# rainerzufalldererste/simd_dct

Hardware: AMD Instinct MI355X
Metric: Mpixels/s 8x8 fwd+inv int16 DCT, 8192x8192 plane (higher is better)
Workload: dtype f32

## Files before the change

simd_dct_amd/csrc/batch_plan.h:

```cpp
#ifndef MDCT_BATCH_PLAN_H
#define MDCT_BATCH_PLAN_H

#include <stddef.h>
#include <stdint.h>

#include <vector>

#include "mdct.h"

#if defined(__HIPCC__)
#define MDCT_HD __host__ __device__ __forceinline__
#else
#define MDCT_HD inline
#endif

namespace mdct
{

struct BatchDesc
{
  const void *from;
  void *to;
  uint64_t pitch_in, pitch_out;
  uint32_t bpr;
  uint32_t tiles;
  uint32_t tiles_m, tiles_s;
  uint32_t first;
  uint32_t table;
  uint32_t has_lut;
  uint32_t rows;
};
static_assert(sizeof(BatchDesc) == 64, "one s_load_dwordx16");
constexpr uint32_t kDescLut = 1, kDescPaired = 2;

struct MagicDiv
{
  uint32_t m, s;
};
inline MagicDiv magic_div(uint32_t d)
{
  if (d <= 1)
    return MagicDiv{0, 0};
  uint32_t l = 0;
  while ((1ull << l) < d)
    l++;
  const uint64_t m = ((1ull << 32) * ((1ull << l) - d)) / d + 1;
  return MagicDiv{(uint32_t)m, 1u | ((l - 1) << 8)};
}
MDCT_HD uint32_t magic_apply(uint32_t n, uint32_t m, uint32_t s)
{
  const uint32_t t = (uint32_t)(((uint64_t)n * m) >> 32);
  return (t + ((n - t) >> (s & 0xFF))) >> (s >> 8);
}

constexpr int kBatchChain = 8;
constexpr uint32_t kBatchMaxTiles = 0xFFFFFFFFu / 64;

template <class FirstOf>
MDCT_HD uint32_t batch_plane_of(uint32_t w, uint32_t n, uint32_t uniform, uint32_t pp_m, uint32_t pp_s, const uint32_t (&first8)[kBatchChain], FirstOf first_of)
{
  if (uniform)
    return magic_apply(w, pp_m, pp_s);
  uint32_t p = 0;
  for (int i = 1; i < kBatchChain; i++)
    p += w >= first8[i] ? 1u : 0u;
  if (n > (uint32_t)kBatchChain)
  {
    uint32_t lo = 0, hi = n;
    while (hi - lo > 1)
    {
      const uint32_t mid = (lo + hi) >> 1;
      if (first_of(mid) <= w)
        lo = mid;
      else
        hi = mid;
    }
    p = lo;
  }
  return p;
}

struct BatchLayout
{
  std::vector<BatchDesc> descs;
  std::vector<int> plane;
  std::vector<int> tables;
  uint32_t total = 0;
  uint32_t uniform = 0;
  uint32_t per_plane = 0;
  MagicDiv pp{0, 0};
  uint32_t first8[kBatchChain];
  int with_lut = 0;
  int consumed = 0;
};

inline uint64_t batch_tiles_of(uint64_t bpr, uint64_t rows, bool paired)
{
  return paired ? (rows / 2) * (bpr / 32) + (rows & 1) * ((bpr + 63) / 64) : ((bpr + 63) / 64) * rows;
}

struct BatchPos
{
  uint32_t row, b0, s, straddle;
};
MDCT_HD BatchPos batch_pos(uint32_t lt, uint32_t bpr, uint32_t tiles, uint32_t tiles_m, uint32_t tiles_s, uint32_t flags, uint32_t rows)
{
  const uint32_t u = magic_apply(lt, tiles_m, tiles_s), blk0 = (lt - u * tiles) * 64;
  BatchPos p;
  if (!(flags & kDescPaired))
  {
    p.row = u;
    p.b0 = blk0;
    p.s = bpr - blk0 < 64u ? bpr - blk0 : 64u;
    p.straddle = 0;
    return p;
  }
  const uint32_t second = blk0 >= bpr ? 1u : 0u;
  p.row = 2 * u + second;
  p.b0 = second ? blk0 - bpr : blk0;
  p.s = bpr - p.b0 < 64u ? bpr - p.b0 : 64u;
  p.straddle = (!second && p.s < 64u && p.row + 1 < rows) ? 1u : 0u;
  return p;
}

template <class Plane>
inline void batch_layout(const Plane *planes, const int *table_id, const unsigned char *has_lut, int i0, int n, size_t blob_bytes, size_t table_size, BatchLayout &out,
                         bool pair_rows = false)
{
  out = BatchLayout();
  uint64_t run = 0;
  for (int i = i0; i < n; i++)
  {
    const Plane &p = planes[i];
    const uint64_t bpr = p.sizeX / 8, rows = p.sizeY / 8;
    if (bpr == 0 || rows == 0)
    {
      out.consumed++;
      continue;
    }
    const bool paired = pair_rows && bpr % 64 == 32 && rows >= 2 && (uint64_t)p.pitch_in < (1ull << 26) && (uint64_t)p.pitch_out < (1ull << 26);
    const uint64_t tiles = paired ? bpr / 32 : (bpr + 63) / 64;
    if (bpr > 0xFFFFFFFFull || rows > 0xFFFFFFFFull || ((bpr + 63) / 64) * rows / rows != (bpr + 63) / 64)
      break;
    const uint64_t mine = batch_tiles_of(bpr, rows, paired);
    if (run + mine > kBatchMaxTiles)
      break;
    int slot = -1;
    bool new_table = false;
    if (table_id[i] >= 0)
    {
      for (size_t k = 0; k < out.tables.size() && slot < 0; k++)
        if (out.tables[k] == table_id[i])
          slot = (int)k;
      new_table = slot < 0;
      if (new_table)
        slot = (int)out.tables.size();
    }
    if (blob_bytes && (out.tables.size() + (new_table ? 1 : 0)) * table_size + (out.descs.size() + 1) * sizeof(BatchDesc) > blob_bytes)
      break;
    if (new_table)
      out.tables.push_back(table_id[i]);
    BatchDesc d;
    d.from = p.from;
    d.to = p.to;
    d.pitch_in = p.pitch_in;
    d.pitch_out = p.pitch_out;
    d.bpr = (uint32_t)bpr;
    d.tiles = (uint32_t)tiles;
    const MagicDiv md = magic_div(d.tiles);
    d.tiles_m = md.m;
    d.tiles_s = md.s;
    d.first = (uint32_t)run;
    d.table = slot < 0 ? 0u : (uint32_t)(slot * table_size);
    d.has_lut = (has_lut[i] ? kDescLut : 0u) | (paired ? kDescPaired : 0u);
    d.rows = (uint32_t)rows;
    out.with_lut += has_lut[i] ? 1 : 0;
    out.descs.push_back(d);
    out.plane.push_back(i);
    out.consumed++;
    run += mine;
  }
  out.total = (uint32_t)run;
  const size_t nd = out.descs.size();
  out.uniform = nd > 0;
  auto tiles_of = [&](size_t k) { return batch_tiles_of(out.descs[k].bpr, out.descs[k].rows, (out.descs[k].has_lut & kDescPaired) != 0); };
  for (size_t k = 1; k < nd; k++)
    if (tiles_of(k) != tiles_of(0))
      out.uniform = 0;
  out.per_plane = out.uniform ? (uint32_t)tiles_of(0) : 0;
  out.pp = magic_div(out.per_plane);
  for (int k = 0; k < kBatchChain; k++)
    out.first8[k] = (size_t)k < nd ? out.descs[k].first : 0xFFFFFFFFu;
}

struct BatchWhere
{
  uint32_t p, row, tile;
  BatchPos pos;
};
inline BatchWhere batch_locate(const BatchDesc *descs, uint32_t n, uint32_t uniform, MagicDiv pp, const uint32_t (&first8)[kBatchChain], uint32_t w)
{
  const uint32_t p = batch_plane_of(w, n, uniform, pp.m, pp.s, first8, [descs](uint32_t k) { return descs[k].first; });
  const BatchDesc &d = descs[p];
  const BatchPos pos = batch_pos(w - d.first, d.bpr, d.tiles, d.tiles_m, d.tiles_s, d.has_lut, d.rows);
  return BatchWhere{p, pos.row, pos.b0 / 64, pos};
}

}
#endif
```

simd_dct_amd/csrc/mdct_api.hip:

```cpp
#include <hip/hip_runtime.h>

#include <cmath>
#include <cstdarg>
#include <cstdio>
#include <cstring>
#include <cxxabi.h>
#include <dlfcn.h>
#include <cstdlib>
#include <string>
#include <mutex>
#include <type_traits>
#include <unordered_map>
#include <vector>

#include "mdct.h"
#include "mdct_kernels.h"
#include "own_tables.h"

namespace
{

thread_local char g_err[512] = "";

int fail(int code, const char *fmt, ...)
// ... 607 lines not shown
        return fail(MDCT_INVALID_PARAMETER, "output strip pitch %zu must be >= 8*sizeX = %zu and a multiple of 16", p.pitch_out, 8 * p.sizeX);
      const uintptr_t in0 = (uintptr_t)p.from, in1 = in0 + (p.sizeY ? (p.sizeY - 1) * p.pitch_in + p.sizeX : 0);
      const uintptr_t out0 = (uintptr_t)p.to, out1 = out0 + (p.sizeY >= 8 ? (p.sizeY / 8 - 1) * p.pitch_out + 8 * p.sizeX : 0);
      if (in0 < out1 && out0 < in1)
        return fail(MDCT_INVALID_PARAMETER, "plane %d: the q32 product cannot be written over its own input (to overlaps from)", i);
      float q[64];
      q32_pair_table(p.lut, false, q);
      q32_safe = q32_safe || table_needs_safe(q);
    }
  for (int i = 0; i < n; i++)
  {
    const Plane &p = planes[i];
    int r;
    if constexpr (U8 || GEN)
      r = u8_plane_args(p.from, p.to, p.pitch_in, p.pitch_out, p.sizeX, p.sizeY, 0, p.sizeY / 8);
    else
      r = own_plane_args(p.from, p.to, sizeof(int16_t), p.pitch_in, p.pitch_out, p.sizeX, p.sizeY, 0, p.sizeY / 8);
    if (r)
      return r;
    if constexpr (GEN)
    {
      const bool fwd = mode == kModeFwdU8;
      if ((((uintptr_t)(fwd ? p.to : p.from)) | ((fwd ? p.pitch_out : p.pitch_in) * sizeof(int16_t))) & 15)
        return fail(MDCT_INVALID_PARAMETER, "coefficient rows must be 16-byte aligned");
    }
    in.has_lut[i] = p.lut != nullptr;
    in.bounded[i] = q32 ? !q32_safe : (U8 ? u8_table_is_tame(p.lut) : (GEN ? (mode == kModeFwdU8 && u8_table_is_bounded(p.lut)) : lut_bounded(p.lut)));
    if (rt && !p.lut)
      continue;
    int id = -1;
    for (size_t k = 0; k < src.size() && id < 0; k++)
      if (src[k] == p.lut || (src[k] && p.lut && memcmp(src[k], p.lut, 64 * sizeof(float)) == 0))
        id = (int)k;
    if (id < 0)
    {
      mdct::OwnTables tb;
      if (q32)
      {
        memset(&tb, 0, sizeof(tb));
        q32_pair_table(p.lut, !q32_safe, tb.qf);
      }
      else if ((r = make_own_tables(p.lut, tb, rt || U8 || GEN)))
        return r;
      id = (int)src.size();
      src.push_back(p.lut);
      in.tables.push_back(tb);
    }
    in.table_id[i] = id;
  }
  return MDCT_SUCCESS;
}

struct BatchLaunch
{
  mdct::BatchArgs args;
  uint32_t total;
  int lutmode;
  bool sat;
};

void batch_header(const mdct::BatchLayout &lay, const BatchInput &in, BatchLaunch &l)
{
  mdct::BatchArgs &a = l.args;
  a.consts = mdct::DctConsts();
  memset(a.px, 0, sizeof(a.px));
  a.pk = pk_consts(true, false);
  memset(&a.head, 0, sizeof(a.head));
  a.head.n = (uint32_t)lay.descs.size();
  a.head.uniform = lay.uniform;
  a.head.pp_m = lay.pp.m;
  a.head.pp_s = lay.pp.s;
  a.head.table_bytes = (uint32_t)(lay.tables.size() * sizeof(mdct::OwnTables));
  memcpy(a.head.first8, lay.first8, sizeof(a.head.first8));
  a.descs = nullptr;
  a.tables = nullptr;
  l.total = lay.total;
  l.lutmode = lay.with_lut == 0 ? mdct::BATCH_NO_LUT : (lay.with_lut == (int)lay.descs.size() ? mdct::BATCH_ALL_LUT : mdct::BATCH_MIXED);
  bool all_bounded = true;
  for (int i : lay.plane)
    all_bounded = all_bounded && in.bounded[i];
  l.sat = !all_bounded;
}

void u8_px_consts(int level_shift, float (&px)[4])
{
  const float shift = level_shift ? 128.0f : 0.0f;
  px[0] = 64.0f * shift;
  px[1] = shift;
  px[2] = px[3] = 0.0f;
}

hipError_t launch_batch(const BatchLaunch &l, int mode, hipStream_t s)
{
  if (mode == kModeQ32)
    return mdct::launch_q32_batch(l.args, l.total, l.sat, s);
  return is_u8_mode(mode) ? mdct::launch_u8_batch(l.args, l.total, mode - kModeRoundtripU8, l.sat, s) : mdct::launch_i16_batch(l.args, l.total, mode, l.lutmode, l.sat, s);
}

template <class Plane>
int run_batch(int mode, const Plane *planes, int n, int level_shift, void *stream)
{
  BatchInput in;
  int r = batch_input(mode, planes, n, in);
  if (r)
    return r;
  const mdct_device_info *di;
  if ((r = current(&di)))
    return r;
  for (int i0 = 0; i0 < n;)
  {
    mdct::BatchLayout lay;
    mdct::batch_layout(planes, in.table_id.data(), in.has_lut.data(), i0, n, mdct::kBatchBlob, sizeof(mdct::OwnTables), lay, pairs_rows(mode));
    if (lay.consumed == 0)
      return fail(MDCT_NOT_SUPPORTED, "plane %d (%zux%zu) exceeds the limit of 2^26 - 1 tiles per launch; split it", i0, planes[i0].sizeX, planes[i0].sizeY);
    i0 += lay.consumed;
    BatchLaunch l;
    batch_header(lay, in, l);
    u8_px_consts(level_shift, l.args.px);
    for (size_t k = 0; k < lay.tables.size(); k++)
      memcpy(l.args.blob + k * sizeof(mdct::OwnTables), &in.tables[lay.tables[k]], sizeof(mdct::OwnTables));
    std::vector<TableRef> parked(lay.tables.size());
    bool all_parked = !lay.tables.empty();
    for (size_t k = 0; k < lay.tables.size() && all_parked; k++)
      all_parked = (parked[k] = table_acquire(di->device, in.tables[lay.tables[k]], (hipStream_t)stream)).dev != nullptr;
    if (all_parked)
    {
      const mdct::OwnTables *base = parked[0].dev;
      for (size_t k = 1; k < parked.size(); k++)
        base = parked[k].dev < base ? parked[k].dev : base;
      l.args.tables = base;
      for (mdct::BatchDesc &d : lay.descs)
        d.table = (uint32_t)((parked[d.table / sizeof(mdct::OwnTables)].dev - base) * sizeof(mdct::OwnTables));
    }
    memcpy(l.args.blob + l.args.head.table_bytes, lay.descs.data(), lay.descs.size() * sizeof(mdct::BatchDesc));
    const hipError_t e = launch_batch(l, mode, (hipStream_t)stream);
    for (const TableRef &r : parked)
      table_release(r, (hipStream_t)stream, all_parked && e == hipSuccess);
    if (e != hipSuccess)
      return hip_fail(e, "plane batch launch");
  }
  return MDCT_SUCCESS;
}

int run_i16_batch(int mode, const mdct_plane_i16 *planes, int n, void *stream) { return run_batch(mode, planes, n, 0, stream); }

}

extern "C" {

int mdct_init(int device)
{
  const hipError_t e = hipSetDevice(device);
  if (e != hipSuccess)
    return hip_fail(e, "hipSetDevice");
  const mdct_device_info *di;
  const int r = current(&di);
  if (r != MDCT_SUCCESS)
    return r;
  (void)mdct::preload_kernels();
  (void)mdct::preload_stage_kernels();
  return MDCT_SUCCESS;
}

int mdct_get_device_info(mdct_device_info *info)
{
  if (!info)
    return fail(MDCT_INVALID_PARAMETER, "null info");
  int dev = 0;
  const hipError_t e = hipGetDevice(&dev);
  if (e != hipSuccess)
    return hip_fail(e, "hipGetDevice");
  const mdct_device_info *di;
  const int r = probe(dev, &di);
  if (r)
    return r;
  *info = *di;
  return MDCT_SUCCESS;
}

const char *mdct_last_error(void) { return g_err; }

static int fwd_quant_u8(const uint8_t *from, uint8_t *to, size_t pitch_in, size_t pitch_out, const float *lut, size_t sizeX, size_t sizeY, size_t by0, size_t by1, int layout, int profile, void *stream)
{
  if (from == nullptr || to == nullptr || lut == nullptr)
    return fail(MDCT_INVALID_PARAMETER, "null pointer");
  const bool combo = (layout == MDCT_LAYOUT_Q32 && profile == MDCT_PROFILE_REF_AVX) || (layout == MDCT_LAYOUT_STEREO && (profile == MDCT_PROFILE_REF_SSE || profile == MDCT_PROFILE_REF_SCALAR)) ||
                     (layout == MDCT_LAYOUT_BLOCK && profile == MDCT_PROFILE_REF_SCALAR) || (layout == MDCT_LAYOUT_BLOCK_SSE && profile == MDCT_PROFILE_REF_SSE);
  if (!combo)
    return fail(MDCT_NOT_SUPPORTED, "layout %d with profile %d is not a reference tier", layout, profile);
  const size_t xmul = layout == MDCT_LAYOUT_Q32 ? 64 : ((profile == MDCT_PROFILE_REF_SSE) ? 16 : 8);
  const size_t ymul = layout == MDCT_LAYOUT_STEREO ? 16 : 8;
  if (sizeX == 0 || sizeX % xmul != 0 || sizeY % ymul != 0)
    return fail(MDCT_NOT_SUPPORTED, "plane %zux%zu: width must be a multiple of %zu and height of %zu for this layout", sizeX, sizeY, xmul, ymul);
  if (pitch_in < sizeX || by0 > by1 || by1 > sizeY / ymul)
    return fail(MDCT_INVALID_PARAMETER, "bad pitch or block-row range [%zu,%zu) for %zu rows", by0, by1, sizeY / ymul);
  if (pitch_out != 0 && layout != MDCT_LAYOUT_Q32 && layout != MDCT_LAYOUT_BLOCK)
    return fail(MDCT_NOT_SUPPORTED, "an output strip pitch exists for the Q32 and BLOCK layouts only");
  if (pitch_out != 0 && (pitch_out < 8 * sizeX || pitch_out % 16 != 0))
    return fail(MDCT_INVALID_PARAMETER, "output strip pitch %zu must be >= 8*sizeX = %zu and a multiple of 16", pitch_out, 8 * sizeX);

  const mdct_device_info *di;
  int r = current(&di);
  if (r)
    return r;

  mdct::U8Args a;
  memset(&a, 0, sizeof(a));
  a.consts = mdct::DctConsts();
  a.from = from;
  a.to = to;
  constexpr float vr = .95f;
  for (int i = 0; i < 64; i++)
    a.qt.q[i] = profile == MDCT_PROFILE_REF_SCALAR ? 1.f / (lut[i] * vr) : 255.0f / (lut[i] * vr);
  const bool safe = profile != MDCT_PROFILE_REF_SCALAR && table_needs_safe(a.qt.q);
  {
    static const int pa[4] = {0, 2, 1, 5}, pb[4] = {4, 6, 3, 7};
    const bool q32 = layout == MDCT_LAYOUT_Q32;
// ... 174 lines not shown
}

int mdct_fwd_i16_jpeg_scan(const int16_t *from, size_t pitch, const float *lut, size_t sizeX, size_t sizeY, size_t by0, size_t by1, int chroma, uint8_t *seg_work, size_t seg_stride, uint64_t *row_work,
                           int first_rst, uint8_t *out, size_t out_capacity, uint64_t *row_offsets, void *stream)
{
  const PxScanOut pack = {row_work, first_rst, out, out_capacity, row_offsets};
  return run_px_huffman(from, true, pitch, lut, 0, sizeX, sizeY, by0, by1, chroma, seg_work, seg_stride, nullptr, nullptr, &pack, stream);
}

int mdct_fwd_u8_i16(const uint8_t *from, int16_t *to, size_t pitch_in, size_t pitch_out, const float *lut, int level_shift, size_t sizeX, size_t sizeY, size_t by0, size_t by1, void *stream)
{
  return run_fwd_u8_i16(from, to, pitch_in, pitch_out, lut, level_shift, sizeX, sizeY, by0, by1, stream);
}

int mdct_inv_i16_u8(const int16_t *from, uint8_t *to, size_t pitch_in, size_t pitch_out, const float *lut, int level_shift, size_t sizeX, size_t sizeY, size_t by0, size_t by1, void *stream)
{
  const int r = u8_i16_plane_args(to, from, pitch_out, pitch_in, sizeX, sizeY, by0, by1);
  if (r)
    return r;
  const GenPlane strip = {from + by0 * 8 * pitch_in, to + by0 * 8 * pitch_out, pitch_in, pitch_out, sizeX, (by1 - by0) * 8, lut};
  return run_batch(kModeInvU8, &strip, 1, level_shift, stream);
}

int mdct_fwd_f32(const float *from, float *to, size_t pitch_in, size_t pitch_out, size_t sizeX, size_t sizeY, size_t by0, size_t by1, void *stream)
{
  return run_f32(mdct::MODE_FWD, from, to, pitch_in, pitch_out, sizeX, sizeY, by0, by1, stream);
}

int mdct_inv_f32(const float *from, float *to, size_t pitch_in, size_t pitch_out, size_t sizeX, size_t sizeY, size_t by0, size_t by1, void *stream)
{
  return run_f32(mdct::MODE_INV, from, to, pitch_in, pitch_out, sizeX, sizeY, by0, by1, stream);
}

int mdct_roundtrip_i16_planes(const mdct_plane_i16 *planes, int n_planes, void *stream) { return run_i16_batch(mdct::MODE_ROUNDTRIP, planes, n_planes, stream); }

int mdct_fwd_i16_batch(const mdct_plane_i16 *planes, int n_planes, void *stream) { return run_i16_batch(mdct::MODE_FWD, planes, n_planes, stream); }
int mdct_inv_i16_batch(const mdct_plane_i16 *planes, int n_planes, void *stream) { return run_i16_batch(mdct::MODE_INV, planes, n_planes, stream); }
int mdct_roundtrip_i16_batch(const mdct_plane_i16 *planes, int n_planes, void *stream) { return run_i16_batch(mdct::MODE_ROUNDTRIP, planes, n_planes, stream); }

struct mdct_batch
{
  int mode = 0, device = 0, n_planes = 0;
  void *dev = nullptr;
  std::vector<BatchLaunch> launches;
};

}

template <class Plane>
static int batch_create(mdct_batch **out, int mode, const Plane *planes, int n_planes, int level_shift)
{
  if (out == nullptr)
    return fail(MDCT_INVALID_PARAMETER, "null batch handle");
  *out = nullptr;
  BatchInput in;
  int r = batch_input(mode, planes, n_planes, in);
  if (r)
    return r;
  const mdct_device_info *di;
  if ((r = current(&di)))
    return r;
  mdct_batch *b = new mdct_batch;
  b->mode = mode;
  b->device = di->device;
  b->n_planes = n_planes;
  std::vector<unsigned char> image;
  std::vector<size_t> at;
  for (int i0 = 0; i0 < n_planes;)
  {
    mdct::BatchLayout lay;
    mdct::batch_layout(planes, in.table_id.data(), in.has_lut.data(), i0, n_planes, 0, sizeof(mdct::OwnTables), lay, pairs_rows(mode));
    if (lay.consumed == 0)
    {
      delete b;
      return fail(MDCT_NOT_SUPPORTED, "plane %d (%zux%zu) exceeds the limit of 2^26 - 1 tiles per launch; split it", i0, planes[i0].sizeX, planes[i0].sizeY);
    }
    i0 += lay.consumed;
    if (lay.descs.empty())
      continue;
    BatchLaunch l;
    batch_header(lay, in, l);
    u8_px_consts(level_shift, l.args.px);
    memset(l.args.blob, 0, sizeof(l.args.blob));
    at.push_back(image.size());
    for (int id : lay.tables)
    {
      const unsigned char *t = reinterpret_cast<const unsigned char *>(&in.tables[id]);
      image.insert(image.end(), t, t + sizeof(mdct::OwnTables));
    }
    const unsigned char *d = reinterpret_cast<const unsigned char *>(lay.descs.data());
    image.insert(image.end(), d, d + lay.descs.size() * sizeof(mdct::BatchDesc));
    b->launches.push_back(l);
  }
  if (!image.empty())
  {
    hipError_t e = hipMalloc(&b->dev, image.size());
    if (e == hipSuccess)
      e = hipMemcpy(b->dev, image.data(), image.size(), hipMemcpyHostToDevice);
    if (e != hipSuccess)
    {
      if (b->dev)
        (void)hipFree(b->dev);
      delete b;
      return hip_fail(e, "plane batch: descriptor table");
    }
    for (size_t k = 0; k < b->launches.size(); k++)
    {
      mdct::BatchArgs &a = b->launches[k].args;
      unsigned char *base = static_cast<unsigned char *>(b->dev) + at[k];
      a.tables = reinterpret_cast<const mdct::OwnTables *>(base);
      a.descs = reinterpret_cast<const mdct::BatchDesc *>(base + a.head.table_bytes);
    }
  }
  *out = b;
  return MDCT_SUCCESS;
}

extern "C" {

int mdct_batch_create(mdct_batch **out, int mode, const mdct_plane_i16 *planes, int n_planes) { return batch_create(out, mode, planes, n_planes, 0); }
int mdct_batch_create_u8(mdct_batch **out, const mdct_plane_u8 *planes, int n_planes, int level_shift) { return batch_create(out, kModeRoundtripU8, planes, n_planes, level_shift); }

int mdct_roundtrip_u8_batch(const mdct_plane_u8 *planes, int n_planes, int level_shift, void *stream) { return run_batch(kModeRoundtripU8, planes, n_planes, level_shift, stream); }

int mdct_fwd_quant32_u8_batch(const mdct_plane_u8 *planes, int n_planes, void *stream) { return run_batch(kModeQ32, planes, n_planes, 0, stream); }
int mdct_batch_create_q32(mdct_batch **out, const mdct_plane_u8 *planes, int n_planes) { return batch_create(out, kModeQ32, planes, n_planes, 0); }

}

static int gen_planes(const mdct_plane_u8_i16 *planes, int n, bool fwd, std::vector<GenPlane> &out)
{
  if (n < 0 || (planes == nullptr && n > 0))
    return fail(MDCT_INVALID_PARAMETER, "null plane list");
  out.resize(n > 0 ? n : 0);
  for (int i = 0; i < n; i++)
  {
    const mdct_plane_u8_i16 &p = planes[i];
    out[i] = fwd ? GenPlane{p.px, p.coef, p.pitch_px, p.pitch_coef, p.sizeX, p.sizeY, p.lut} : GenPlane{p.coef, p.px, p.pitch_coef, p.pitch_px, p.sizeX, p.sizeY, p.lut};
  }
  return MDCT_SUCCESS;
}

namespace mdct
{
TallySlot g_tally[kTallySlots];
}

namespace
{
std::mutex g_tally_mu;
const char *g_tally_names[mdct::kTallySlots];

const char *tally_name(size_t slot, const void *kernel)
{
  std::lock_guard<std::mutex> lk(g_tally_mu);
  if (g_tally_names[slot] != nullptr)
    return g_tally_names[slot];
  std::string name;
  Dl_info info;
  if (dladdr(kernel, &info) != 0 && info.dli_sname != nullptr && info.dli_saddr == kernel)
  {
    int st = 0;
    char *d = abi::__cxa_demangle(info.dli_sname, nullptr, nullptr, &st);
    name = st == 0 && d != nullptr ? d : info.dli_sname;
    std::free(d);
    if (name.compare(0, 5, "void ") == 0)
// ... 239 lines not shown
```

simd_dct_amd/csrc/mdct_kernels.h:

```cpp
#ifndef MDCT_KERNELS_H
#define MDCT_KERNELS_H

#include <hip/hip_runtime.h>
#include <stddef.h>
#include <stdint.h>

#include "mdct.h"
#include "batch_plan.h"
#include "launch_tally.h"

namespace mdct
{

enum { MODE_FWD = 0, MODE_INV = 1, MODE_ROUNDTRIP = 2 };

struct DctConsts
{
  float c707 = 0.707106781186547524f;
  float c382 = 0.382683432365089772f;
  float c541 = 0.541196100146196985f;
  float c1306 = 1.306562964876376528f;
  float c1414 = 1.414213562373095049f;
  float c1847 = 1.847759065022573512f;
  float c1082 = 1.082392200292393968f;
// ... 41 lines not shown
  size_t eye_offset;
  size_t plane_stride;
  uint32_t bpr;
  uint32_t by0;
  uint32_t by_last;
  uint32_t nblocks;
  uint32_t spill_ok;
  uint32_t out_tight;
};

struct I16Args
{
  const int16_t *from;
  int16_t *to;
  const OwnTables *tb_dev;
  OwnTables tb;
  DctConsts consts;
  size_t pitch_in, pitch_out;
  uint32_t bpr, by0, nblocks;
};

struct U8I16Args
{
  const uint8_t *px;
  int16_t *coef;
  OwnTables tb;
  DctConsts consts;
  size_t pitch_px, pitch_coef;
  uint32_t bpr, by0, nblocks;
  float dc_shift;
};

struct U8RecArgs
{
  const uint8_t *px;
  int16_t *levels;
  uint8_t *runs;
  uint8_t *counts;
  OwnTables tb;
  DctConsts consts;
  size_t pitch_px;
  uint32_t bpr, by0, nblocks;
  float dc_shift;
};

struct PxHuffArgs
{
  const uint8_t *px;
  uint8_t *out;
  uint32_t *seg_bytes;
  uint32_t *ff_counts;
  size_t seg_stride;
  size_t pitch_px;
  OwnTables tb;
  DctConsts consts;
  uint32_t bpr, by0;
  float dc_shift;
  uint32_t dc[12];
  uint32_t ac[256];
  uint8_t *scan;
  unsigned long long capacity;
  unsigned long long *row_off;
  unsigned long long *work;
  uint32_t n_rows, first_rst;
};

struct F32Args
{
  const float *from;
  float *to;
  float scale[64];
  DctConsts consts;
  size_t pitch_in, pitch_out;
  uint32_t bpr, by0, nblocks;
};

constexpr int kBatchBlob = 3584;
struct BatchHead
{
  uint32_t n;
  uint32_t uniform;
  uint32_t pp_m, pp_s;
  uint32_t table_bytes;
  uint32_t pad[3];
  uint32_t first8[kBatchChain];
};
static_assert(sizeof(BatchHead) == 64, "one s_load_dwordx16");
struct BatchArgs
{
  BatchHead head;
  const BatchDesc *descs;
  const OwnTables *tables;
  DctConsts consts;
  alignas(8) float px[4];
  PkConstsArg pk;
  alignas(64) unsigned char blob[kBatchBlob];
};
static_assert(offsetof(BatchArgs, descs) == 64 && offsetof(BatchArgs, tables) == 72, "the batch kernels read head + pointers as 20 consecutive dwords");
static_assert(offsetof(BatchArgs, px) % 8 == 0, "k_u8_batch reads px as two register pairs");
static_assert(sizeof(BatchArgs) <= 4096, "kernel argument block");
enum { BATCH_NO_LUT = 0, BATCH_ALL_LUT = 1, BATCH_MIXED = 2 };
hipError_t launch_i16_batch(const BatchArgs &a, uint32_t total, int mode, int lutmode, bool sat, hipStream_t s);
hipError_t launch_u8_batch(const BatchArgs &a, uint32_t total, int mode, bool general, hipStream_t s);
hipError_t launch_q32_batch(const BatchArgs &a, uint32_t total, bool safe, hipStream_t s);

hipError_t launch_fwd_quant_u8(const U8Args &a, int layout, int profile, bool safe, hipStream_t s);
hipError_t launch_i16(const I16Args &a, int mode, bool has_lut, hipStream_t s, bool lut_bounded = false);
hipError_t launch_u8_i16_fwd(const U8I16Args &a, hipStream_t s);
hipError_t launch_u8_records(const U8RecArgs &a, bool i16_in, hipStream_t s, bool clamp = true);
hipError_t launch_px_huffman(const PxHuffArgs &a, bool i16_in, bool pack, bool clamp, uint32_t n_rows, hipStream_t s);
hipError_t launch_f32(const F32Args &a, int mode, hipStream_t s);
hipError_t launch_park_table(const OwnTables &tb, OwnTables *slot, hipStream_t s);
hipError_t launch_clock_probe(unsigned long long *out, unsigned int ticks, unsigned int waves, hipStream_t s);
hipError_t preload_kernels();
hipError_t preload_stage_kernels();
hipError_t launch_stream_copy(const void *from, void *to, size_t bytes, int cus, hipStream_t s);

}
#endif
```

simd_dct_amd/csrc/mdct_kernels.hip:

```cpp
#include <hip/hip_runtime.h>
#include <stddef.h>
#include <stdint.h>
#include <stdlib.h>

#include <type_traits>

#include "wg_sync.h"
#include "huffman_rows.h"
#include "pack_rows.h"
#include "mdct_kernels.h"
#include "scan_records.h"
#include "aan_passes.h"

#pragma clang fp contract(off)

namespace mdct
{


enum { K_AVX = 0, K_SSE = 1, K_TRUE = 2 };

__device__ __forceinline__ void aan_fwd8(const DctConsts &C, float &p0, float &p1, float &p2, float &p3, float &p4, float &p5, float &p6, float &p7)
{
  const float t0 = p0 + p7, t7 = p0 - p7, t1 = p1 + p6, t6 = p1 - p6;
// ... 650 lines not shown
  }
  else
  {
    if (valid)
    {
      const uint32_t ab = bx & 1;
      uint32_t L[8];
#pragma unroll
      for (int i8 = 0; i8 < 8; i8++)
        L[i8] = pack4_lo8(q[i8 * 8 + 0], q[i8 * 8 + 1], q[i8 * 8 + 4], q[i8 * 8 + 5]);
      uint32_t w[8];
#pragma unroll
      for (int j = 0; j < 4; j++)
      {
        const uint32_t keep = ab ? L[4 + j] : L[j], give = ab ? L[j] : L[4 + j];
        const uint32_t got = (uint32_t)__builtin_amdgcn_mov_dpp((int)give, 0xB1 , 0xF, 0xF, true);
        w[2 * j] = ab ? got : keep;
        w[2 * j + 1] = ab ? keep : got;
      }
      uint8_t *pair = a.to + (size_t)by * 8 * a.sizeX + (size_t)(bx >> 1) * 128;
      typedef unsigned int u32x4_unaligned __attribute__((ext_vector_type(4), aligned(1)));
      const u32x4_unaligned v0 = {w[0], w[1], w[2], w[3]}, v1 = {w[4], w[5], w[6], w[7]};
      if constexpr (TILED)
      {
        const gptr_t wg_out = sgpr_ptr(a.to + (size_t)by * 8 * a.sizeX + (size_t)(blockIdx.x * kWG) * 64);
        const uint32_t off = (threadIdx.x >> 1) * 128 + ab * 32;
        *reinterpret_cast<u32x4_unaligned __attribute__((address_space(1))) *>(wg_out + off) = v0;
        *reinterpret_cast<u32x4_unaligned __attribute__((address_space(1))) *>(wg_out + off + 16) = v1;
      }
      else
      {
        *reinterpret_cast<u32x4_unaligned *>(pair + ab * 32) = v0;
        *reinterpret_cast<u32x4_unaligned *>(pair + ab * 32 + 16) = v1;
      }
      const bool spill = (by == a.by_last) && ((bx | 1u) == a.bpr - 1) && a.spill_ok;
      if (spill)
      {
#pragma unroll
        for (int i8 = 0; i8 < 8; i8++)
          *reinterpret_cast<uint32_t *>(pair + ab * 4 + 128 + i8 * 8) = pack4_lo8(q[i8 * 8 + 2], q[i8 * 8 + 3], q[i8 * 8 + 6], q[i8 * 8 + 7]);
      }
    }
  }
}

typedef unsigned int u32x4 __attribute__((ext_vector_type(4)));
typedef float f32x4 __attribute__((ext_vector_type(4)));

__device__ __forceinline__ uint4 ld_stream16(const void *p)
{
  const u32x4 v = __builtin_nontemporal_load(reinterpret_cast<const u32x4 *>(p));
  return make_uint4(v.x, v.y, v.z, v.w);
}

__device__ __forceinline__ void st_stream16(void *p, uint32_t x, uint32_t y, uint32_t z, uint32_t w)
{
  const u32x4 v = {x, y, z, w};
  __builtin_nontemporal_store(v, reinterpret_cast<u32x4 *>(p));
}

struct RowsLinear
{
  const int16_t *src;
  int16_t *dst;
  size_t pitch_in, pitch_out;
  __device__ __forceinline__ uint4 ld(int r) const { return ld_stream16(src + (size_t)r * pitch_in); }
  __device__ __forceinline__ void st(int r, uint32_t x, uint32_t y, uint32_t z, uint32_t w) const { st_stream16(dst + (size_t)r * pitch_out, x, y, z, w); }
};
struct RowsTiled
{
  const int16_t *src;
  int16_t *dst;
  size_t pitch_in, pitch_out;
  uint32_t lane_off;
  uint32_t lane_off_out;
  __device__ __forceinline__ uint4 ld(int r) const
  {
    const u32x4_g v = __builtin_nontemporal_load(reinterpret_cast<const u32x4_g __attribute__((address_space(1))) *>(sgpr_ptr(src + (size_t)r * pitch_in) + lane_off));
    return make_uint4(v.x, v.y, v.z, v.w);
  }
  __device__ __forceinline__ void st(int r, uint32_t x, uint32_t y, uint32_t z, uint32_t w) const { store16_g(sgpr_ptr(dst + (size_t)r * pitch_out) + lane_off_out, u32x4_g{x, y, z, w}); }
};

__device__ __forceinline__ void unpack_i16x8(const uint4 v, float (&row)[8])
{
  row[0] = (float)(int16_t)(v.x & 0xFFFF); row[1] = (float)(int16_t)(v.x >> 16);
  row[2] = (float)(int16_t)(v.y & 0xFFFF); row[3] = (float)(int16_t)(v.y >> 16);
  row[4] = (float)(int16_t)(v.z & 0xFFFF); row[5] = (float)(int16_t)(v.z >> 16);
  row[6] = (float)(int16_t)(v.w & 0xFFFF); row[7] = (float)(int16_t)(v.w >> 16);
}

template <int SHIFT>
__device__ __forceinline__ uint32_t rne_i16_bits(const DctConsts &C, float v)
{
  constexpr float scale = (float)(1 << SHIFT);
  const float m = __builtin_amdgcn_fmed3f(v, -32768.0f * scale, 32767.0f * scale);
  return __float_as_uint(m + (SHIFT == 0 ? C.magic23 : C.magic29));
}

__device__ __forceinline__ uint32_t quant_i16_bits(const DctConsts &C, float y, float qf)
{
  return __float_as_uint(__builtin_amdgcn_fmed3f(__builtin_fmaf(y, qf, C.magic23), kQLo, kQHi));
}
__device__ __forceinline__ float quant_i16_float(const DctConsts &C, float y, float qf)
{
  return __builtin_amdgcn_fmed3f(__builtin_fmaf(y, qf, C.magic23), kQLo, kQHi) - C.magic23;
}

__device__ __forceinline__ uint32_t pack_lo16(uint32_t lo, uint32_t hi) { return __builtin_amdgcn_perm(hi, lo, 0x05040100u); }

__device__ __forceinline__ void store_q_i16x8(const DctConsts &C, int16_t *dst, const float (&row)[8], const float *qf)
{
  uint32_t t[8];
#pragma unroll
  for (int c = 0; c < 8; c++)
    t[c] = quant_i16_bits(C, row[c], qf[c]);
  st_stream16(dst, pack_lo16(t[0], t[1]), pack_lo16(t[2], t[3]), pack_lo16(t[4], t[5]), pack_lo16(t[6], t[7]));
}

template <int MODE, bool HAS_LUT, class Rows, class Tables>
__device__ __forceinline__ void i16_block(const DctConsts &C, const Rows rows, const Tables &tb)
{
  float b[8][8];
#pragma unroll
  for (int r = 0; r < 8; r++)
    unpack_i16x8(rows.ld(r), b[r]);

  if constexpr (MODE == MODE_INV)
  {
#pragma unroll
    for (int i = 0; i < 64; i++)
      b[i >> 3][i & 7] = b[i >> 3][i & 7] * tb.dq[i];
  }
  else
    raw_fwd(C, b);

  if constexpr (MODE != MODE_FWD)
  {
    if constexpr (MODE == MODE_ROUNDTRIP && HAS_LUT)
    {
#pragma unroll
      for (int i = 0; i < 64; i++)
        b[i >> 3][i & 7] = quant_i16_float(C, b[i >> 3][i & 7], tb.qf[i]) * tb.dq[i];
    }
    raw_inv(C, b);
  }

  constexpr int SHIFT = (MODE == MODE_ROUNDTRIP && !HAS_LUT) ? 6 : 0;
#pragma unroll
  for (int r = 0; r < 8; r++)
  {
    uint32_t t[8];
#pragma unroll
    for (int c = 0; c < 8; c++)
      t[c] = MODE == MODE_FWD ? quant_i16_bits(C, b[r][c], tb.qf[r * 8 + c]) : rne_i16_bits<SHIFT>(C, b[r][c]);
    rows.st(r, pack_lo16(t[0], t[1]), pack_lo16(t[2], t[3]), pack_lo16(t[4], t[5]), pack_lo16(t[6], t[7]));
  }
}

__device__ __forceinline__ void quant_dequant8(const AanPk &K, f32x2 (&p)[8], const f32x2 (&qf)[8], const f32x2 (&dq)[8])
{
#define MDCT_Q8(OP, A, B, MOD) OP " %0, %0, " A "0" B MOD OP " %1, %1, " A "1" B MOD OP " %2, %2, " A "2" B MOD OP " %3, %3, " A "3" B MOD OP " %4, %4, " A "4" B MOD OP " %5, %5, " A "5" B MOD OP " %6, %6, " A "6" B MOD OP " %7, %7, " A "7" B MOD
  asm("v_pk_fma_f32 %0, %0, %8, %24 op_sel:[0,0,0] op_sel_hi:[1,1,0]\n\t"
      "v_pk_fma_f32 %1, %1, %9, %24 op_sel:[0,0,0] op_sel_hi:[1,1,0]\n\t"
      "v_pk_fma_f32 %2, %2, %10, %24 op_sel:[0,0,0] op_sel_hi:[1,1,0]\n\t"
      "v_pk_fma_f32 %3, %3, %11, %24 op_sel:[0,0,0] op_sel_hi:[1,1,0]\n\t"
// ... 97 lines not shown
  constexpr float scale = HAS_LUT ? 1.0f : 64.0f;
#pragma unroll
  for (int r = 0; r < 8; r++)
  {
    f32x2 o07, o16, o25, o43;
    aan_inv_h(K, P[0][r], P[1][r], P[2][r], P[3][r], o07, o16, o25, o43);
    auto fin = [&](f32x2 v) {
      f32x2 t;
      v.x = __builtin_amdgcn_fmed3f(v.x, -32768.0f * scale, 32767.0f * scale);
      v.y = __builtin_amdgcn_fmed3f(v.y, -32768.0f * scale, 32767.0f * scale);
      if constexpr (HAS_LUT)
        MDCT_PKA(t, v, K.magic, MDCT_K_LL);
      else
        MDCT_PKA(t, v, K.magic, MDCT_K_HH);
      return t;
    };
    const f32x2 b07 = fin(o07), b16 = fin(o16), b25 = fin(o25), b43 = fin(o43);
    rows.st(r, pack_lo16(__float_as_uint(b07.x), __float_as_uint(b16.x)), pack_lo16(__float_as_uint(b25.x), __float_as_uint(b43.y)),
            pack_lo16(__float_as_uint(b43.x), __float_as_uint(b25.y)), pack_lo16(__float_as_uint(b16.y), __float_as_uint(b07.y)));
  }
}

typedef const __attribute__((address_space(4))) OwnTables *ktables_t;
__device__ __forceinline__ kbytes_t i16_tables(const I16Args &a) { return a.tb_dev ? const_bytes(a.tb_dev) : karg_bytes(offsetof(I16Args, tb)); }

constexpr int i16_waves(int mode) { return mode == MODE_ROUNDTRIP ? 3 : (mode == MODE_FWD ? 2 : 4); }
template <int MODE, bool HAS_LUT, bool SAT = true>
__global__ __launch_bounds__(kWG) __attribute__((amdgpu_waves_per_eu(i16_waves(MODE), i16_waves(MODE)))) void k_i16(I16Args a)
{
  const uint32_t t = wg_index() * kWG + threadIdx.x;
  if (t >= a.nblocks)
    return;
  const uint32_t row = t / a.bpr;
  const uint32_t bx = t - row * a.bpr;
  const size_t by = a.by0 + row;
  const int16_t *src = a.from + by * 8 * a.pitch_in + (size_t)bx * 8;
  int16_t *dst = a.to + by * 8 * a.pitch_out + (size_t)bx * 8;
  const kbytes_t tbp = i16_tables(a);
  if constexpr (MODE == MODE_ROUNDTRIP)
    i16_roundtrip_rows<HAS_LUT, RowsLinear, false, SAT>(a.consts, RowsLinear{src, dst, a.pitch_in, a.pitch_out}, tbp);
  else
    i16_block<MODE, HAS_LUT>(a.consts, RowsLinear{src, dst, a.pitch_in, a.pitch_out}, *(ktables_t)tbp);
}

constexpr uint32_t kTileSmallLaunch = 6144;
template <int MODE, bool HAS_LUT, bool SAT = true, int WAVES = 2>
__global__ __launch_bounds__(64) __attribute__((amdgpu_waves_per_eu(WAVES, WAVES))) void k_i16_tile(I16Args a)
{
  const size_t by = a.by0 + blockIdx.y;
  const RowsTiled rows{a.from + by * 8 * a.pitch_in + (size_t)blockIdx.x * 512, a.to + by * 8 * a.pitch_out + (size_t)blockIdx.x * 512, a.pitch_in, a.pitch_out, threadIdx.x * 16, threadIdx.x * 16};
  const kbytes_t tbp = i16_tables(a);
  if constexpr (MODE == MODE_ROUNDTRIP)
    i16_roundtrip_rows<HAS_LUT, RowsTiled, true, SAT>(a.consts, rows, tbp);
  else
    i16_block<MODE, HAS_LUT>(a.consts, rows, *(ktables_t)tbp);
}

typedef uint32_t u32x16_s __attribute__((ext_vector_type(16)));
typedef uint32_t u32x4_s __attribute__((ext_vector_type(4)));
static_assert(offsetof(BatchDesc, from) == 0 && offsetof(BatchDesc, to) == 8 && offsetof(BatchDesc, pitch_in) == 16 && offsetof(BatchDesc, pitch_out) == 24 && offsetof(BatchDesc, bpr) == 32 &&
                  offsetof(BatchDesc, tiles) == 36 && offsetof(BatchDesc, tiles_m) == 40 && offsetof(BatchDesc, tiles_s) == 44 && offsetof(BatchDesc, first) == 48 && offsetof(BatchDesc, table) == 52 &&
                  offsetof(BatchDesc, has_lut) == 56,
              "batch_tile picks the descriptor's fields out of one 16-dword load");

struct BatchTile
{
  u32x16_s d;
  uint32_t row;
  uint32_t tile;
  uint32_t b0, s, straddle;
  kbytes_t tables;
  __device__ __forceinline__ uint32_t bpr() const { return d[8]; }
  __device__ __forceinline__ uint32_t has_lut() const { return d[14] & kDescLut; }
  __device__ __forceinline__ uint64_t from() const { return ((uint64_t)d[1] << 32) | d[0]; }
  __device__ __forceinline__ uint64_t to() const { return ((uint64_t)d[3] << 32) | d[2]; }
  __device__ __forceinline__ size_t pitch_in() const { return ((uint64_t)d[5] << 32) | d[4]; }
  __device__ __forceinline__ size_t pitch_out() const { return ((uint64_t)d[7] << 32) | d[6]; }
};
template <bool PAIRS = false>
__device__ __forceinline__ BatchTile batch_tile(uint32_t w)
{
  kbytes_t args = karg_bytes(0);
  asm volatile("" : "+s"(args));
  const u32x16_s h = *(const __attribute__((address_space(4))) u32x16_s *)args;
  const u32x4_s ptrs = *(const __attribute__((address_space(4))) u32x4_s *)(args + offsetof(BatchArgs, descs));
  const uint32_t n = h[0], uniform = h[1], pp_m = h[2], pp_s = h[3], table_bytes = h[4];
  const uint64_t descs_dev = ((uint64_t)ptrs[1] << 32) | ptrs[0], tables_dev = ((uint64_t)ptrs[3] << 32) | ptrs[2];
  const kbytes_t blob = args + offsetof(BatchArgs, blob);
  const kbytes_t descs = descs_dev ? (kbytes_t)descs_dev : blob + table_bytes;
  const kbytes_t tables = tables_dev ? (kbytes_t)tables_dev : blob;
  const uint32_t first8[kBatchChain] = {h[8], h[9], h[10], h[11], h[12], h[13], h[14], h[15]};
  static_assert(kBatchChain == 8 && offsetof(BatchHead, first8) == 32, "first8 = dwords 8..15 of the header");
  uint32_t p = batch_plane_of(w, n, uniform, pp_m, pp_s, first8, [descs](uint32_t k) {
    return *(const __attribute__((address_space(4))) uint32_t *)(descs + (size_t)k * sizeof(BatchDesc) + offsetof(BatchDesc, first));
  });
  p = __builtin_amdgcn_readfirstlane(p);
  kbytes_t dp = descs + (size_t)p * sizeof(BatchDesc);
  asm volatile("" : "+s"(dp));
  BatchTile t;
  t.d = *(const __attribute__((address_space(4))) u32x16_s *)dp;
  const uint32_t lt = w - t.d[12];
  if constexpr (PAIRS)
  {
    const BatchPos at = batch_pos(lt, t.d[8], t.d[9], t.d[10], t.d[11], t.d[14], t.d[15]);
    t.row = at.row, t.b0 = at.b0, t.s = at.s, t.straddle = at.straddle, t.tile = at.b0 >> 6;
  }
  else
  {
    t.row = magic_apply(lt, t.d[10], t.d[11]);
    t.tile = lt - t.row * t.d[9];
    t.b0 = t.tile * 64, t.s = 64, t.straddle = 0;
  }
  t.tables = tables + t.d[13];
  return t;
}

constexpr int batch_waves(int mode) { return mode == MODE_ROUNDTRIP ? 3 : 2; }
template <int MODE, int LUTMODE, bool SAT = true, bool SMALL = false>
__global__ __launch_bounds__(64) __attribute__((amdgpu_waves_per_eu(SMALL ? 4 : batch_waves(MODE), SMALL ? 4 : batch_waves(MODE)))) void k_i16_batch(BatchArgs a)
{
  const BatchTile t = batch_tile<true>(blockIdx.x);
  if (!t.straddle && threadIdx.x >= t.s)
    return;
  const size_t pin = t.pitch_in(), pout = t.pitch_out();
  const uint32_t hop = (t.straddle && threadIdx.x >= t.s) ? 0xFFFFFFFFu : 0u;
  const RowsTiled rows{(const int16_t *)t.from() + (size_t)t.row * 8 * pin + (size_t)t.b0 * 8, (int16_t *)t.to() + (size_t)t.row * 8 * pout + (size_t)t.b0 * 8, pin, pout,
                       threadIdx.x * 16 + (hop & (((uint32_t)pin - t.bpr()) * 16)), threadIdx.x * 16 + (hop & (((uint32_t)pout - t.bpr()) * 16))};
  if constexpr (MODE == MODE_ROUNDTRIP)
  {
    if (LUTMODE == BATCH_ALL_LUT || (LUTMODE == BATCH_MIXED && t.has_lut()))
      i16_roundtrip_rows<true, RowsTiled, true, SAT>(a.consts, rows, t.tables);
    else
      i16_roundtrip_rows<false, RowsTiled, true>(a.consts, rows, nullptr);
  }
  else
    i16_block<MODE, true>(a.consts, rows, *(ktables_t)t.tables);
}

__device__ __forceinline__ uint32_t pack4_sat_u8(float x0, float x1, float x2, float x3)
{
  uint32_t w = __builtin_amdgcn_cvt_pk_u8_f32(x0, 0, 0u);
  w = __builtin_amdgcn_cvt_pk_u8_f32(x1, 1, w);
  w = __builtin_amdgcn_cvt_pk_u8_f32(x2, 2, w);
  return __builtin_amdgcn_cvt_pk_u8_f32(x3, 3, w);
}
enum { U8_RT = 0, U8_FWD = 1, U8_INV = 2 };
template <int MODE, bool SAT, bool PRIO>
__device__ __forceinline__ void u8_rows(const DctConsts &C, const f32x2 shifts, const void *src, void *dst, size_t pitch_in, size_t pitch_out, uint32_t in_off, uint32_t out_off, kbytes_t tbp)
{
  const AanPk &K = reinterpret_cast<const AanPk &>(C);
  f32x2 P[4][8];
  if constexpr (MODE != U8_INV)
  {
    uint2 rows[8];
    load_block_rows_g(static_cast<const uint8_t *>(src), pitch_in, in_off, rows);
    MDCT_PHASE_PRIO(1);
#pragma unroll
    for (int r = 0; r < 8; r++)
    {
      const f32x2 a01 = {ubyte_to_float<0>(rows[r].x), ubyte_to_float<1>(rows[r].x)}, a23 = {ubyte_to_float<2>(rows[r].x), ubyte_to_float<3>(rows[r].x)};
      const f32x2 a45 = {ubyte_to_float<0>(rows[r].y), ubyte_to_float<1>(rows[r].y)}, a67 = {ubyte_to_float<2>(rows[r].y), ubyte_to_float<3>(rows[r].y)};
      aan_fwd_h(K, a01, a23, a45, a67, P[0][r], P[1][r], P[2][r], P[3][r]);
    }
  }
  else
  {
    const RowsTiled in{static_cast<const int16_t *>(src), nullptr, pitch_in, 0, in_off, 0};
    uint4 rows[8];
#pragma unroll
    for (int v = 0; v < 8; v++)
      rows[v] = in.ld(v);
    MDCT_PHASE_PRIO(1);
#pragma unroll
    for (int v = 0; v < 8; v++)
    {
      const uint4 w = rows[v];
      P[0][v] = f32x2{(float)(int16_t)(w.x & 0xFFFF), (float)(int16_t)(w.z & 0xFFFF)};
      P[1][v] = f32x2{(float)(int16_t)(w.y & 0xFFFF), (float)(int16_t)(w.w & 0xFFFF)};
      P[2][v] = f32x2{(float)(int16_t)(w.z >> 16), (float)(int16_t)(w.y >> 16)};
      P[3][v] = f32x2{(float)(int16_t)(w.x >> 16), (float)(int16_t)(w.w >> 16)};
    }
  }
  MDCT_PHASE_PRIO(2);
#pragma unroll
  for (int j = 0; j < 4; j++)
  {
    karg_pairs_t tq = (karg_pairs_t)(tbp + offsetof(OwnTables, qf)) + j * 8, td = (karg_pairs_t)(tbp + offsetof(OwnTables, dq)) + j * 8;
    asm volatile("" : "+s"(tq), "+s"(td));
    if constexpr (MODE != U8_INV)
    {
      aan_fwd_v(K, P[j]);
      if (j == 0)
        P[0][0].x = P[0][0].x - shifts.x;
    }
    if constexpr (MODE == U8_RT)
      quant_dequant_pairs<SAT>(K, P[j], tq, td);
    else if constexpr (MODE == U8_FWD)
    {
      const f32x2 magic_v = K.magic;
#pragma unroll
      for (int v = 0; v < 8; v++)
      {
        f32x2 m;
        MDCT_PKF(m, P[j][v], tq[v], magic_v, "op_sel:[0,0,0] op_sel_hi:[1,1,0]");
        if constexpr (SAT)
        {
          m.x = __builtin_amdgcn_fmed3f(m.x, kQLo, kQHi);
          m.y = __builtin_amdgcn_fmed3f(m.y, kQLo, kQHi);
        }
        P[j][v] = m;
      }
    }
    else
    {
#pragma unroll
      for (int v = 0; v < 8; v++)
// ... 874 lines not shown
```

Measured before the change: 1.554 million.

## Embed up to three plane descriptors in kernel args and chain row pointers

Adds a copy of up to three batch descriptors to the kernel argument block so the batch kernel picks its descriptor with two compares from preloaded scalar registers. This replaces the dependent scalar load of the descriptor table. The i16 batch kernel now walks rows with incrementing SGPR pointers and nontemporal loads, instead of recomputing row*pitch addresses each time. This enlarges the argument block and adds three extra s_load_dwordx16 per workgroup. Nontemporal loads may also change cache behaviour.

```diff
diff --git a/simd_dct_amd/csrc/batch_plan.h b/simd_dct_amd/csrc/batch_plan.h
--- a/simd_dct_amd/csrc/batch_plan.h
+++ b/simd_dct_amd/csrc/batch_plan.h
@@ -80,6 +80,13 @@
   return p;
 }
 
+constexpr int kBatchCopies = 3;
+MDCT_HD uint32_t batch_plane_of_copies(uint32_t w, const uint32_t (&first8)[kBatchChain])
+{
+  static_assert(kBatchCopies == 3 && kBatchCopies <= kBatchChain, "two compares");
+  return w < first8[1] ? 0u : (w < first8[2] ? 1u : 2u);
+}
+
 struct BatchLayout
 {
   std::vector<BatchDesc> descs;
@@ -115,12 +122,17 @@
     p.straddle = 0;
     return p;
   }
-  const uint32_t second = blk0 >= bpr ? 1u : 0u;
-  p.row = 2 * u + second;
+  const bool second = blk0 >= bpr;
+  p.row = second ? 2 * u + 1 : 2 * u;
   p.b0 = second ? blk0 - bpr : blk0;
   p.s = bpr - p.b0 < 64u ? bpr - p.b0 : 64u;
   p.straddle = (!second && p.s < 64u && p.row + 1 < rows) ? 1u : 0u;
   return p;
+}
+
+MDCT_HD uint64_t batch_row_bytes(uint32_t units, uint64_t pitch)
+{
+  return (uint64_t)units * (uint32_t)pitch + ((uint64_t)(units * (uint32_t)(pitch >> 32)) << 32);
 }
 
 template <class Plane>
@@ -193,6 +205,17 @@
     out.first8[k] = (size_t)k < nd ? out.descs[k].first : 0xFFFFFFFFu;
 }
 
+inline bool batch_copies(const BatchLayout &lay, BatchDesc (&copies)[kBatchCopies])
+{
+  for (int k = 0; k < kBatchCopies; k++)
+    copies[k] = BatchDesc{};
+  if (lay.descs.empty() || lay.descs.size() > (size_t)kBatchCopies)
+    return false;
+  for (size_t k = 0; k < lay.descs.size(); k++)
+    copies[k] = lay.descs[k];
+  return true;
+}
+
 struct BatchWhere
 {
   uint32_t p, row, tile;
diff --git a/simd_dct_amd/csrc/mdct_api.hip b/simd_dct_amd/csrc/mdct_api.hip
--- a/simd_dct_amd/csrc/mdct_api.hip
+++ b/simd_dct_amd/csrc/mdct_api.hip
@@ -713,6 +713,12 @@
   l.sat = !all_bounded;
 }
 
+void batch_attach_copies(const mdct::BatchLayout &lay, BatchLaunch &l)
+{
+  if (mdct::batch_copies(lay, l.args.copies))
+    l.args.head.flags |= mdct::kHeadCopies;
+}
+
 void u8_px_consts(int level_shift, float (&px)[4])
 {
   const float shift = level_shift ? 128.0f : 0.0f;
@@ -764,6 +770,7 @@
         d.table = (uint32_t)((parked[d.table / sizeof(mdct::OwnTables)].dev - base) * sizeof(mdct::OwnTables));
     }
     memcpy(l.args.blob + l.args.head.table_bytes, lay.descs.data(), lay.descs.size() * sizeof(mdct::BatchDesc));
+    batch_attach_copies(lay, l);
     const hipError_t e = launch_batch(l, mode, (hipStream_t)stream);
     for (const TableRef &r : parked)
       table_release(r, (hipStream_t)stream, all_parked && e == hipSuccess);
@@ -1104,6 +1111,7 @@
     batch_header(lay, in, l);
     u8_px_consts(level_shift, l.args.px);
     memset(l.args.blob, 0, sizeof(l.args.blob));
+    batch_attach_copies(lay, l);
     at.push_back(image.size());
     for (int id : lay.tables)
     {
diff --git a/simd_dct_amd/csrc/mdct_kernels.h b/simd_dct_amd/csrc/mdct_kernels.h
--- a/simd_dct_amd/csrc/mdct_kernels.h
+++ b/simd_dct_amd/csrc/mdct_kernels.h
@@ -147,10 +147,12 @@
   uint32_t uniform;
   uint32_t pp_m, pp_s;
   uint32_t table_bytes;
-  uint32_t pad[3];
+  uint32_t flags;
+  uint32_t pad[2];
   uint32_t first8[kBatchChain];
 };
 static_assert(sizeof(BatchHead) == 64, "one s_load_dwordx16");
+constexpr uint32_t kHeadCopies = 1;
 struct BatchArgs
 {
   BatchHead head;
@@ -160,9 +162,11 @@
   alignas(8) float px[4];
   PkConstsArg pk;
   alignas(64) unsigned char blob[kBatchBlob];
+  alignas(64) BatchDesc copies[kBatchCopies];
 };
 static_assert(offsetof(BatchArgs, descs) == 64 && offsetof(BatchArgs, tables) == 72, "the batch kernels read head + pointers as 20 consecutive dwords");
 static_assert(offsetof(BatchArgs, px) % 8 == 0, "k_u8_batch reads px as two register pairs");
+static_assert(offsetof(BatchArgs, copies) == offsetof(BatchArgs, blob) + kBatchBlob && offsetof(BatchArgs, copies) % 64 == 0, "appended after the existing fields");
 static_assert(sizeof(BatchArgs) <= 4096, "kernel argument block");
 enum { BATCH_NO_LUT = 0, BATCH_ALL_LUT = 1, BATCH_MIXED = 2 };
 hipError_t launch_i16_batch(const BatchArgs &a, uint32_t total, int mode, int lutmode, bool sat, hipStream_t s);
diff --git a/simd_dct_amd/csrc/mdct_kernels.hip b/simd_dct_amd/csrc/mdct_kernels.hip
--- a/simd_dct_amd/csrc/mdct_kernels.hip
+++ b/simd_dct_amd/csrc/mdct_kernels.hip
@@ -756,6 +756,26 @@
   __device__ __forceinline__ void st(int r, uint32_t x, uint32_t y, uint32_t z, uint32_t w) const { store16_g(sgpr_ptr(dst + (size_t)r * pitch_out) + lane_off_out, u32x4_g{x, y, z, w}); }
 };
 
+struct RowsChained
+{
+  mutable gptr_t src, dst;
+  uint64_t step_in, step_out;
+  uint32_t lane_off, lane_off_out;
+  __device__ __forceinline__ uint4 ld(int) const
+  {
+    const u32x4_g v = __builtin_nontemporal_load(reinterpret_cast<const u32x4_g __attribute__((address_space(1))) *>(src + lane_off));
+    src += step_in;
+    asm("" : "+s"(src));
+    return make_uint4(v.x, v.y, v.z, v.w);
+  }
+  __device__ __forceinline__ void st(int, uint32_t x, uint32_t y, uint32_t z, uint32_t w) const
+  {
+    store16_g(dst + lane_off_out, u32x4_g{x, y, z, w});
+    dst += step_out;
+    asm("" : "+s"(dst));
+  }
+};
+
 __device__ __forceinline__ void unpack_i16x8(const uint4 v, float (&row)[8])
 {
   row[0] = (float)(int16_t)(v.x & 0xFFFF); row[1] = (float)(int16_t)(v.x >> 16);
@@ -1019,23 +1039,36 @@
 {
   kbytes_t args = karg_bytes(0);
   asm volatile("" : "+s"(args));
-  const u32x16_s h = *(const __attribute__((address_space(4))) u32x16_s *)args;
-  const u32x4_s ptrs = *(const __attribute__((address_space(4))) u32x4_s *)(args + offsetof(BatchArgs, descs));
+  u32x16_s h = *(const __attribute__((address_space(4))) u32x16_s *)args;
+  u32x4_s ptrs = *(const __attribute__((address_space(4))) u32x4_s *)(args + offsetof(BatchArgs, descs));
+  u32x16_s c0 = *(const __attribute__((address_space(4))) u32x16_s *)(args + offsetof(BatchArgs, copies));
+  u32x16_s c1 = *(const __attribute__((address_space(4))) u32x16_s *)(args + offsetof(BatchArgs, copies) + sizeof(BatchDesc));
+  u32x16_s c2 = *(const __attribute__((address_space(4))) u32x16_s *)(args + offsetof(BatchArgs, copies) + 2 * sizeof(BatchDesc));
+  static_assert(kBatchCopies == 3, "three copies, one s_load_dwordx16 each");
+  asm volatile("" : "+s"(h), "+s"(ptrs), "+s"(c0), "+s"(c1), "+s"(c2));
   const uint32_t n = h[0], uniform = h[1], pp_m = h[2], pp_s = h[3], table_bytes = h[4];
   const uint64_t descs_dev = ((uint64_t)ptrs[1] << 32) | ptrs[0], tables_dev = ((uint64_t)ptrs[3] << 32) | ptrs[2];
   const kbytes_t blob = args + offsetof(BatchArgs, blob);
   const kbytes_t descs = descs_dev ? (kbytes_t)descs_dev : blob + table_bytes;
   const kbytes_t tables = tables_dev ? (kbytes_t)tables_dev : blob;
   const uint32_t first8[kBatchChain] = {h[8], h[9], h[10], h[11], h[12], h[13], h[14], h[15]};
-  static_assert(kBatchChain == 8 && offsetof(BatchHead, first8) == 32, "first8 = dwords 8..15 of the header");
-  uint32_t p = batch_plane_of(w, n, uniform, pp_m, pp_s, first8, [descs](uint32_t k) {
-    return *(const __attribute__((address_space(4))) uint32_t *)(descs + (size_t)k * sizeof(BatchDesc) + offsetof(BatchDesc, first));
-  });
-  p = __builtin_amdgcn_readfirstlane(p);
-  kbytes_t dp = descs + (size_t)p * sizeof(BatchDesc);
-  asm volatile("" : "+s"(dp));
+  static_assert(kBatchChain == 8 && offsetof(BatchHead, first8) == 32 && offsetof(BatchHead, flags) == 20, "first8 = dwords 8..15 of the header, flags = dword 5");
   BatchTile t;
-  t.d = *(const __attribute__((address_space(4))) u32x16_s *)dp;
+  if (h[5] & kHeadCopies)
+  {
+    const uint32_t p = batch_plane_of_copies(w, first8);
+    t.d = p == 0 ? c0 : (p == 1 ? c1 : c2);
+  }
+  else
+  {
+    uint32_t p = batch_plane_of(w, n, uniform, pp_m, pp_s, first8, [descs](uint32_t k) {
+      return *(const __attribute__((address_space(4))) uint32_t *)(descs + (size_t)k * sizeof(BatchDesc) + offsetof(BatchDesc, first));
+    });
+    p = __builtin_amdgcn_readfirstlane(p);
+    kbytes_t dp = descs + (size_t)p * sizeof(BatchDesc);
+    asm volatile("" : "+s"(dp));
+    t.d = *(const __attribute__((address_space(4))) u32x16_s *)dp;
+  }
   const uint32_t lt = w - t.d[12];
   if constexpr (PAIRS)
   {
@@ -1061,14 +1094,14 @@
     return;
   const size_t pin = t.pitch_in(), pout = t.pitch_out();
   const uint32_t hop = (t.straddle && threadIdx.x >= t.s) ? 0xFFFFFFFFu : 0u;
-  const RowsTiled rows{(const int16_t *)t.from() + (size_t)t.row * 8 * pin + (size_t)t.b0 * 8, (int16_t *)t.to() + (size_t)t.row * 8 * pout + (size_t)t.b0 * 8, pin, pout,
-                       threadIdx.x * 16 + (hop & (((uint32_t)pin - t.bpr()) * 16)), threadIdx.x * 16 + (hop & (((uint32_t)pout - t.bpr()) * 16))};
+  const RowsChained rows{sgpr_ptr((const char *)t.from() + batch_row_bytes(t.row * 16, pin) + (size_t)t.b0 * 16), sgpr_ptr((char *)t.to() + batch_row_bytes(t.row * 16, pout) + (size_t)t.b0 * 16), pin * 2, pout * 2,
+                         threadIdx.x * 16 + (hop & (((uint32_t)pin - t.bpr()) * 16)), threadIdx.x * 16 + (hop & (((uint32_t)pout - t.bpr()) * 16))};
   if constexpr (MODE == MODE_ROUNDTRIP)
   {
     if (LUTMODE == BATCH_ALL_LUT || (LUTMODE == BATCH_MIXED && t.has_lut()))
-      i16_roundtrip_rows<true, RowsTiled, true, SAT>(a.consts, rows, t.tables);
+      i16_roundtrip_rows<true, RowsChained, true, SAT>(a.consts, rows, t.tables);
     else
-      i16_roundtrip_rows<false, RowsTiled, true>(a.consts, rows, nullptr);
+      i16_roundtrip_rows<false, RowsChained, true>(a.consts, rows, nullptr);
   }
   else
     i16_block<MODE, true>(a.consts, rows, *(ktables_t)t.tables);
```

Result: no change. 1.557 million (median of 3 runs) (+0.2%).
